# Corleno/Nonstationary_Multivariate_Gaussian_Process

Measured on AMD Instinct MI355X. Metric: log-posterior evals/sec (N=2048, D=3 nonseparable GP), higher is better.
Workload: dtype f64

## Files before the change

nonstationary_multivariate_gaussian_process_amd/csrc/nmgp_chol.hip:

```cpp
#include "nmgp_internal.h"
#include <cstring>

namespace nmgpk {

static inline int cdiv_c(long long a, long long b) { return (int)((a + b - 1) / b); }

typedef double v4d __attribute__((ext_vector_type(4)));

#define SY_BM 128
#define SY_BK 16
#define SY_LD (SY_BM + 16)
#define SY_SB 8

__device__ __forceinline__ int clamp_row_pair(int r, int rows) {
    int rc = r < rows - 1 ? r : rows - 2;
    return rc < 0 ? 0 : rc;
}

__device__ __forceinline__ double fast_recip(double p) {
    double x = __builtin_amdgcn_rcp(p);
    double e = fma(-p, x, 1.0);
    x = fma(x, e, x);
    e = fma(-p, x, 1.0);
    x = fma(x, e, x);
// ... 1445 lines not shown
#pragma unroll
        for (int kk = 0; kk < 4; ++kk) x0 = __builtin_amdgcn_mfma_f64_16x16x4f64(ai[kk], T[pp][kk], x0, 0, 0, 0);
        T[pp] = x0;
#pragma unroll
        for (int kk = 0; kk < 4; ++kk)
#pragma unroll
            for (int q = pp + 1; q < 4; ++q) {
                const double a = reinterpret_cast<const double*>(&ops[(q == 1 ? 0 : (q == 2 ? 1 : 3)) + pp][lane])[kk];
                T[q] = __builtin_amdgcn_mfma_f64_16x16x4f64(a, T[pp][kk], T[q], 0, 0, 0);
            }
    }
    if (v0) {
#pragma unroll
        for (int q = 0; q < 4; ++q)
#pragma unroll
            for (int r = 0; r < 4; ++r) A[(size_t)(16 * q + 4 * r + l4) * lda + row] = T[q][r];
    }
}

static void trsm_64(hipStream_t s, const double* L, int ldl, int nb, double* A, int lda, int rows, int batch,
                    long long bstride, bool precise) {
    if (rows <= 0) return;
    if (precise) {
        NMGP_LAUNCH(k_trsm_64, dim3(cdiv_c(rows, 64), batch), dim3(256), 0, s, L, ldl, nb, A, lda, rows, bstride);
    } else if (nb == 64) {
        NMGP_LAUNCH(k_trsm_64h<5>, dim3(cdiv_c(rows, 64), batch), dim3(256), 0, s, L, ldl, A, lda, rows, bstride);
    } else {
        const long long wgs = (long long)cdiv_c(rows, 128) * batch;
        const int reps = wgs >= 4096 ? 4 : (wgs >= 2048 ? 2 : 1);
        NMGP_LAUNCH(k_trsm_64m, dim3(cdiv_c(rows, 128 * reps), batch), dim3(256), 0, s, L, ldl, nb, A, lda, rows, bstride, reps);
    }
}

#define PS_XLD 66
#define PS_XPS_OFF 6656
#define PS_XS_OFF (PS_XPS_OFF + 64 * PS_XLD)
#define PS_SMEM_DOUBLES (PS_XS_OFF + 64 * PS_XLD)

template <int MODE, int OCC = 2>
__global__ __launch_bounds__(512, OCC) void k_panel_step(double* __restrict__ Ab, int lda, int ck, int has_prev_a,
                                                        int has_next_a,
                                                        int m_act, int pend, long long bstride, int* __restrict__ info,
                                                        int istride, int T, int u_mrows, int u_ncols, int u_kflags,
                                                        int u_tiles, int nbatch, int pre_a, int un_fresh, int u_tri,
                                                        long long* __restrict__ stamps) {
    const int has_prev = MODE == 0 ? has_prev_a : (MODE == 2 ? 1 : 0);
    const int has_next = MODE == 0 ? has_next_a : (MODE == 1 ? 1 : 0);
    const int pre = MODE == 0 ? pre_a : 0;
    constexpr int kOpsT = MODE == 1 ? 0 : 4096;
    constexpr int kXps = PS_XPS_OFF;
    constexpr int kXs = MODE == 1 ? 2560 : PS_XS_OFF;
    constexpr int kSmem = MODE == 1 ? 2560 + 64 * PS_XLD
                                    : (MODE == 2 ? 6656 : (PS_SMEM_DOUBLES > 4 * SY_BK * SY_LD ? PS_SMEM_DOUBLES : 4 * SY_BK * SY_LD));
    static_assert(MODE != 1 || sizeof(Potf2Lds) <= kSmem * sizeof(double), "the factorisation's LDS aliases the step's");
#define PS_STAMP(i)                                                              \
    do {                                                                         \
        if (stamps && blockIdx.x == 0 && threadIdx.x == 0) stamps[i] = (long long)wall_clock64(); \
    } while (0)
    PS_STAMP(0);
    __shared__ __attribute__((aligned(32))) double smem[kSmem];
    const int tid = threadIdx.x, lane = tid & 63, w = tid >> 6;
    const int l15 = lane & 15, l4 = lane >> 4;
    const int bx = (int)blockIdx.x / nbatch, by = (int)blockIdx.x - bx * nbatch;
    if (bx >= T) {
        if constexpr (MODE == 0) {
            const int t = bx - T + by * u_tiles;
            const double* Ap = Ab + (size_t)(ck - 64) * lda + (ck + 128);
            double* Cp = Ab + (size_t)(ck + 128) * lda + (ck + 128);
            syrk_tile_body<4, SY_BK>(Ap, lda, Cp, lda, u_mrows, u_ncols, 64, bstride, bstride, u_kflags, -u_tiles, nbatch, t, 0,
                                     0, smem, smem + 2 * SY_BK * SY_LD, u_tri, 0);
        }
        return;
    }
    double* A = Ab + (size_t)by * bstride;
    v4d* opsC = reinterpret_cast<v4d*>(smem);
    v4d* opsT = reinterpret_cast<v4d*>(smem + kOpsT);
    double* Xps = smem + (MODE == 0 ? kXps : 0);
    double* Xs = smem + (MODE == 2 ? 0 : kXs);
    const bool wg0 = bx == 0;
    const bool isC = wg0 && w < 4;
    const bool wg1 = pre && bx == 1;
    const bool isP = wg1 && w < 4;
    const int row = wg0 ? ck + 64 + 16 * w + l15 : ck + 128 + 128 * (bx - 1) + 16 * w + l15;
    const bool rv = row < m_act && !(wg0 && w >= 4);
    const int rowc = row < m_act ? row : (m_act - 1);
    const bool un_used = has_next && (has_prev || wg0);
    double oc[8], ot[5];
    v4d Xp[4], Tk[4], Un[4];
    const double* Lp = A + (size_t)(ck - 64) * lda;
    if (has_prev) {
#pragma unroll
        for (int j = 0; j < 8; ++j) {
            const int e = tid + 512 * j, q = e >> 10, sx = (e >> 6) & 15, l = e & 63;
            oc[j] = -Lp[(size_t)(4 * sx + (l >> 4)) * lda + ck + 16 * q + (l & 15)];
        }
    }
    {
        const double* L = A + (size_t)ck * lda + ck;
#pragma unroll
        for (int j = 0; j < 5; ++j) {
            const int idx = tid + 512 * j;
            const int blk = idx >> 8, kk = (idx >> 6) & 3, l = idx & 63;
            const int rr = l & 15, kc = 4 * kk + (l >> 4);
            double v;
            if (blk < 6) {
                const int q = blk == 0 ? 1 : (blk < 3 ? 2 : 3);
                const int pp = blk == 0 ? 0 : (blk < 3 ? blk - 1 : blk - 3);
                v = -L[(size_t)(16 * pp + kc) * lda + 16 * q + rr];
            } else {
                const int q = blk - 6;
                if (kc < rr) v = L[(size_t)(16 * q + rr) * lda + 16 * q + kc];
                else if (kc == rr) v = 1.0 / L[(size_t)(16 * q + rr) * lda + 16 * q + rr];
                else v = 0.0;
            }
            ot[j] = v;
        }
    }
    auto load_rows = [&]() {
#pragma unroll
        for (int q = 0; q < 4; ++q)
#pragma unroll
            for (int r = 0; r < 4; ++r) {
                const int c = 16 * q + 4 * r + l4;
                Tk[q][r] = rv ? A[(size_t)(ck + c) * lda + rowc] : 0.0;
                Xp[q][r] = (rv && has_prev) ? Lp[(size_t)c * lda + rowc] : 0.0;
                Un[q][r] = (rv && un_used && row < un_fresh) ? A[(size_t)(ck + 64 + c) * lda + rowc] : 0.0;
            }
    };
    if constexpr (MODE != 2) load_rows();
    if (has_prev) {
#pragma unroll
        for (int j = 0; j < 8; ++j) {
            const int e = tid + 512 * j, q = e >> 10, sx = (e >> 6) & 15, l = e & 63;
            smem[((q * 4 + (sx >> 2)) * 64 + l) * 4 + (sx & 3)] = oc[j];
        }
        if (isP) {
#pragma unroll
            for (int q = 0; q < 4; ++q)
#pragma unroll
                for (int r = 0; r < 4; ++r) Xps[(16 * w + l15) * PS_XLD + 16 * q + 4 * r + l4] = Xp[q][r];
        }
    }
#pragma unroll
    for (int j = 0; j < 5; ++j) {
        const int idx = tid + 512 * j;
        const int blk = idx >> 8, kk = (idx >> 6) & 3, l = idx & 63;
        smem[kOpsT + (blk * 64 + l) * 4 + kk] = ot[j];
    }
    if constexpr (MODE == 2) load_rows();
    __syncthreads();
    PS_STAMP(1);
    if (has_prev && has_next && !wg0) {
#pragma unroll
        for (int j = 0; j < 8; ++j) {
            const int e = tid + 512 * j, q = e >> 10, sx = (e >> 6) & 15, l = e & 63;
            oc[j] = -Lp[(size_t)(4 * sx + (l >> 4)) * lda + ck + 64 + 16 * q + (l & 15)];
        }
    }
    if (has_prev && (!wg0 || isC)) {
#pragma unroll
        for (int sg = 0; sg < 4; ++sg)
#pragma unroll
            for (int kk = 0; kk < 4; ++kk)
#pragma unroll
                for (int q = 0; q < 4; ++q) {
                    const double a = reinterpret_cast<const double*>(&opsC[(q * 4 + sg) * 64 + lane])[kk];
                    Tk[q] = __builtin_amdgcn_mfma_f64_16x16x4f64(a, Xp[sg][kk], Tk[q], 0, 0, 0);
                }
    }
    PS_STAMP(2);
#pragma unroll
    for (int pp = 0; pp < 4; ++pp) {
        const v4d ai = opsT[(6 + pp) * 64 + lane];
        v4d x0 = {0.0, 0.0, 0.0, 0.0};
#pragma unroll
        for (int kk = 0; kk < 4; ++kk) x0 = __builtin_amdgcn_mfma_f64_16x16x4f64(ai[kk], Tk[pp][kk], x0, 0, 0, 0);
        Tk[pp] = x0;
#pragma unroll
        for (int kk = 0; kk < 4; ++kk)
#pragma unroll
            for (int q = pp + 1; q < 4; ++q) {
                const double a = reinterpret_cast<const double*>(&opsT[((q == 1 ? 0 : (q == 2 ? 1 : 3)) + pp) * 64 + lane])[kk];
                Tk[q] = __builtin_amdgcn_mfma_f64_16x16x4f64(a, Tk[pp][kk], Tk[q], 0, 0, 0);
            }
    }
    if (rv) {
#pragma unroll
        for (int q = 0; q < 4; ++q)
#pragma unroll
            for (int r = 0; r < 4; ++r) A[(size_t)(ck + 16 * q + 4 * r + l4) * lda + row] = Tk[q][r];
    }
    PS_STAMP(3);
    if (!has_next) return;
    if (!wg0) {
        if (isP) {
#pragma unroll
            for (int q = 0; q < 4; ++q)
#pragma unroll
                for (int r = 0; r < 4; ++r) Xs[(16 * w + l15) * PS_XLD + 16 * q + 4 * r + l4] = Tk[q][r];
        }
        if (wg1 && !has_prev) __syncthreads();
        if (has_prev) {
            __syncthreads();
#pragma unroll
            for (int j = 0; j < 8; ++j) {
                const int e = tid + 512 * j, q = e >> 10, sx = (e >> 6) & 15, l = e & 63;
                smem[((q * 4 + (sx >> 2)) * 64 + l) * 4 + (sx & 3)] = oc[j];
            }
            __syncthreads();
#pragma unroll
            for (int sg = 0; sg < 4; ++sg)
#pragma unroll
                for (int kk = 0; kk < 4; ++kk)
#pragma unroll
                    for (int q = 0; q < 4; ++q) {
                        const double a = reinterpret_cast<const double*>(&opsC[(q * 4 + sg) * 64 + lane])[kk];
                        Un[q] = __builtin_amdgcn_mfma_f64_16x16x4f64(a, Xp[sg][kk], Un[q], 0, 0, 0);
                    }
        }
        if (rv && (has_prev || row >= un_fresh)) {
#pragma unroll
            for (int q = 0; q < 4; ++q)
#pragma unroll
                for (int r = 0; r < 4; ++r) A[(size_t)(ck + 64 + 16 * q + 4 * r + l4) * lda + row] = Un[q][r];
        }
        if (isP) {
#pragma unroll 1
            for (int q0 = 0; q0 < 4; q0 += 2) {
                v4d Vn[2];
#pragma unroll
                for (int qq = 0; qq < 2; ++qq)
#pragma unroll
                    for (int r = 0; r < 4; ++r) Vn[qq][r] = A[(size_t)(ck + 128 + 16 * (q0 + qq) + 4 * r + l4) * lda + rowc];
                if (has_prev) {
#pragma unroll
                    for (int sg = 0; sg < 4; ++sg)
#pragma unroll
                        for (int kk = 0; kk < 4; ++kk)
#pragma unroll
                            for (int qq = 0; qq < 2; ++qq) {
                                const double a = -Xps[(16 * (q0 + qq) + l15) * PS_XLD + 16 * sg + 4 * kk + l4];
                                const double b = Xps[(16 * w + l15) * PS_XLD + 16 * sg + 4 * kk + l4];
                                Vn[qq] = __builtin_amdgcn_mfma_f64_16x16x4f64(a, b, Vn[qq], 0, 0, 0);
                            }
                }
#pragma unroll
                for (int sg = 0; sg < 4; ++sg)
#pragma unroll
                    for (int kk = 0; kk < 4; ++kk)
#pragma unroll
                        for (int qq = 0; qq < 2; ++qq) {
                            const double a = -Xs[(16 * (q0 + qq) + l15) * PS_XLD + 16 * sg + 4 * kk + l4];
                            const double b = Xs[(16 * w + l15) * PS_XLD + 16 * sg + 4 * kk + l4];
                            Vn[qq] = __builtin_amdgcn_mfma_f64_16x16x4f64(a, b, Vn[qq], 0, 0, 0);
                        }
#pragma unroll
                for (int qq = 0; qq < 2; ++qq)
#pragma unroll
                    for (int r = 0; r < 4; ++r) A[(size_t)(ck + 128 + 16 * (q0 + qq) + 4 * r + l4) * lda + row] = Vn[qq][r];
            }
        }
        return;
    }
    if (isC) {
#pragma unroll
        for (int q = 0; q < 4; ++q)
#pragma unroll
            for (int r = 0; r < 4; ++r) Xs[(16 * w + l15) * PS_XLD + 16 * q + 4 * r + l4] = Tk[q][r];
    }
    PS_STAMP(4);
    __syncthreads();
    PS_STAMP(5);
    if (isC) {
#pragma unroll
        for (int sg = 0; sg < 4; ++sg)
#pragma unroll
            for (int kk = 0; kk < 4; ++kk)
#pragma unroll
                for (int q = 0; q < 4; ++q) {
                    const double a = -Xs[(16 * q + l15) * PS_XLD + 16 * sg + 4 * kk + l4];
                    Un[q] = __builtin_amdgcn_mfma_f64_16x16x4f64(a, Tk[sg][kk], Un[q], 0, 0, 0);
                }
    }
    Potf2Lds& P = *reinterpret_cast<Potf2Lds*>(smem);
    __syncthreads();
    if (isC) {
#pragma unroll
        for (int q = 0; q < 4; ++q)
#pragma unroll
            for (int r = 0; r < 4; ++r) {
                const int rr = 16 * w + l15, cc = 16 * q + 4 * r + l4;
                P.S[cc * PB_LD + rr] = (cc <= rr) ? Un[q][r] : 0.0;
            }
    }
    __syncthreads();
    PS_STAMP(6);
    potf2b_core_mfma(P, info + (size_t)by * istride, ck + 64);
    PS_STAMP(7);
    potf2b_store(A + (size_t)(ck + 64) * lda + (ck + 64), lda, 64, P, tid, 512);
    PS_STAMP(8);
#undef PS_STAMP
}

__global__ void k_set_row(double* __restrict__ A, int lda, int row, const double* __restrict__ v, int n,
                          long long bstride, long long vstride, int cps) {
    int j = blockIdx.x * blockDim.x + threadIdx.x;
    if (j < n) A[(size_t)blockIdx.y * bstride + (size_t)j * lda + row] = v[(size_t)(blockIdx.y / cps) * vstride + j];
}
void set_row(hipStream_t s, double* A, int lda, int row, const double* v, int n, int batch, long long bstride,
             long long vstride, int cps) {
    NMGP_LAUNCH(k_set_row, dim3(cdiv_c(n, 256), batch), dim3(256), 0, s, A, lda, row, v, n, bstride, vstride, cps < 1 ? 1 : cps);
}
__global__ void k_get_row(const double* __restrict__ A, int lda, int row, double* __restrict__ v, int n,
                          long long bstride, long long vstride) {
    int j = blockIdx.x * blockDim.x + threadIdx.x;
    if (j < n) v[(size_t)blockIdx.y * vstride + j] = A[(size_t)blockIdx.y * bstride + (size_t)j * lda + row];
}
void get_row(hipStream_t s, const double* A, int lda, int row, double* v, int n, int batch, long long bstride,
             long long vstride) {
    NMGP_LAUNCH(k_get_row, dim3(cdiv_c(n, 256), batch), dim3(256), 0, s, A, lda, row, v, n, bstride, vstride);
}

struct Factorisation {
    hipStream_t s, s2;
    double* A;
    int lda, n, extra, xtri;
    int* info;
    int batch;
    long long bs;
    int is;
    bool precise;
    const SyrkHook* hook;
    long long* stamps;
    bool block_done = false;

    double* at(int row, int col) const { return A + (size_t)col * lda + row; }
    int active_rows(int cend) const { return n + extra + (cend < xtri ? cend : xtri); }
    bool take_block_done() {
        const bool done = block_done;
        block_done = false;
        return done;
    }

    void update(hipStream_t st, int c0, int k, int c1, int ncols, int fuse_width) {
        const bool fuse = fuse_width >= 64 && !precise;
        const bool done = syrk_lower(st, at(c1, c0), lda, at(c1, c1), lda, active_rows(c0 + k) - c1, ncols, k, batch, bs, -1, 0,
                                     xtri > 0 ? n + extra - c1 : kNoTriRows, c0, fuse ? info : nullptr, is, c1, hook);
        if (fuse) block_done = done;
    }

    void block_solve(int c0, int w) {
        if (!take_block_done()) potf2_64(s, at(c0, c0), lda, w, info, c0, batch, bs, is, precise);
        trsm_64(s, at(c0, c0), lda, w, at(c0 + w, c0), lda, active_rows(c0 + w) - (c0 + w), batch, bs, precise);
    }

    void fused_steps(int c0, int w, bool leaf) {
        if (!take_block_done()) potf2_64(s, at(c0, c0), lda, 64, info, c0, batch, bs, is, precise);
        const int nk = w / 64;
        for (int k = 0; k < nk; ++k) {
            const int ck = c0 + 64 * k;
            const int m_act = active_rows(ck + 64);
            const int rows = m_act - (ck + 64);
            if (rows <= 0) continue;
            const int has_prev = k > 0, has_next = k + 1 < nk;
            const int T = 1 + (rows > 64 ? cdiv_c(rows - 64, 128) : 0);
            SyrkPlan pl;
            const int u_m = m_act - (ck + 128), u_n = c0 + w - (ck + 128);
            if (has_prev && u_m > 0 && u_n > 0) pl = syrk_plan(lda, lda, u_m, u_n, 64, 1, 0, true);
            const int pre = (ck + 192 <= c0 + w) ? 1 : 0;
            if (pre) pl.kflags |= 128;
            long long* st = stamps ? stamps + (size_t)(ck / 64) * 16 : nullptr;
            const int un_fresh = xtri > 0 ? n + extra + (has_prev ? ck - 64 : ck) : kNoTriRows;
            const int u_tri = xtri > 0 ? n + extra - 64 * NMGP_XTRI_SEED_BLOCKS : kNoTriRows;
            if (leaf && pl.tiles == 0 && !pre && nk == 2) {
                if (k == 0)
                    NMGP_LAUNCH((k_panel_step<1, 4>), dim3((unsigned)(T * batch)), dim3(512), 0, s, A, lda, ck, 0, 1, m_act, c0 + w, bs, info,
                                is, T, 0, 0, 0, 0, batch, 0, un_fresh, u_tri, st);
                else
                    NMGP_LAUNCH((k_panel_step<2, 6>), dim3((unsigned)(T * batch)), dim3(512), 0, s, A, lda, ck, 1, 0, m_act, c0 + w, bs, info,
                                is, T, 0, 0, 0, 0, batch, 0, un_fresh, u_tri, st);
            } else {
                NMGP_LAUNCH((k_panel_step<0, 2>), dim3((unsigned)((T + pl.tiles) * batch)), dim3(512), 0, s, A, lda, ck, has_prev, has_next, m_act,
                            c0 + w, bs, info, is, T, pl.mrows, u_n, pl.kflags, pl.tiles, batch, pre, un_fresh, u_tri, st);
            }
        }
    }

    void panel_rl(int c0, int w) {
        for (int j0 = c0; j0 < c0 + w; j0 += 64) {
            const int jb = (c0 + w - j0 < 64) ? (c0 + w - j0) : 64;
            block_solve(j0, jb);
            update(s, j0, jb, j0 + jb, c0 + w - (j0 + jb), c0 + w - (j0 + jb));
        }
    }

    enum Leaf {
        kBlockSolve,
        kFusedSteps,
        kLeaf128
    };
    void panel_halving(int c0, int w, int base, Leaf leaf) {
        if (w <= base) {
            if (leaf == kBlockSolve || (leaf == kLeaf128 && w != 128)) block_solve(c0, w);
            else fused_steps(c0, w, leaf == kLeaf128);
            return;
        }
        int h = ((w / 2 + 63) / 64) * 64;
        if (h >= w) h = ((w - 1) / 64) * 64;
        panel_halving(c0, h, base, leaf);
        update(s, c0, h, c0 + h, w - h, w - h);
        panel_halving(c0 + h, w - h, base, leaf);
    }

    void panel(int c0, int w) {
        const Switches& sw = switches();
        const bool mfma_ok = w > 0 && (w % 64 == 0) && (lda % 2 == 0) && !precise;
        const bool small = sw.fused_max_batch >= 0 ? batch <= sw.fused_max_batch : (long long)batch * n <= 73728;
        const int rec_min_batch = 4;
        if (mfma_ok && (sw.panel == Switches::kFused || (sw.panel == Switches::kAuto && small)))
            panel_halving(c0, w, fused_base(w), kFusedSteps);
        else if (mfma_ok && sw.panel == Switches::kAuto && batch >= rec_min_batch && w >= 128)
            panel_halving(c0, w, 128, kLeaf128);
        else if (sw.panel == Switches::kRl || (sw.panel != Switches::kRec && batch < rec_min_batch))
            panel_rl(c0, w);
        else
            panel_halving(c0, w, 64, kBlockSolve);
    }
    int fused_base(int w) const {
        if (switches().fused_base >= 64) return switches().fused_base;
        if (w > 256 && (batch >= 16 || (xtri > 0 && batch >= 5))) return 256;
        return w;
    }

    void run(int nb1, hipEvent_t* ev) {
        const bool la = (s2 != nullptr && ev != nullptr && n > 2 * nb1 && batch <= switches().la_max_batch && !precise);
        if (!la) {
            for (int c0 = 0; c0 < n; c0 += nb1) {
                const int w1 = (n - c0 < nb1) ? (n - c0) : nb1;
                const int c1 = c0 + w1;
                panel(c0, w1);
                update(s, c0, w1, c1, n - c1, n - c1 < nb1 ? n - c1 : nb1);
            }
            return;
        }
        hipEventRecord(ev[0], s);
        hipStreamWaitEvent(s2, ev[0], 0);
        int k = 0;
        bool prevB = false;
        for (int c0 = 0; c0 < n; c0 += nb1, ++k) {
            const int w1 = (n - c0 < nb1) ? (n - c0) : nb1;
            const int c1 = c0 + w1;
            const int w1n = (c1 < n) ? ((n - c1 < nb1) ? (n - c1) : nb1) : 0;
            const int c2 = c1 + w1n;
            hipEvent_t evPanel = ev[1 + 2 * k], evB = ev[2 + 2 * k];
            panel(c0, w1);
            if (c1 >= n) break;
            if (prevB) hipStreamWaitEvent(s, ev[2 + 2 * (k - 1)], 0);
            update(s, c0, w1, c1, w1n, w1n);
            hipEventRecord(evPanel, s);
            prevB = false;
            if (c2 < n) {
                hipStreamWaitEvent(s2, evPanel, 0);
                update(s2, c0, w1, c2, n - c2, 0);
                hipEventRecord(evB, s2);
                prevB = true;
            }
        }
        if (prevB) hipStreamWaitEvent(s, ev[2 + 2 * (k - 1)], 0);
    }
};

void potrf_lower(hipStream_t s, hipStream_t s2, hipEvent_t* ev, double* A, int lda, int n, int extra, int xtri,
                 int nb1, int* info, int batch, long long bstride, int istride, const SyrkHook* hook, int precise) {
    if (nb1 <= 0)
        nb1 = (batch >= 16 && n >= 4096) ? 2048
              : (((batch >= 4 && n >= 4096) || (batch >= 32 && n >= 2048)) && (long long)batch * n > 73728) ? 1024 : 512;
    const int nsteps = (n + 63) / 64;
    Factorisation f{s, s2, A, lda, n, extra, xtri, info, batch, bstride, istride, precise != 0, hook, g_step_stamps.begin(s, nsteps)};
    f.run(nb1, ev);
    g_step_stamps.dump(s, nsteps);
}

static_assert(SY_BM + 2 * SY_BK - 2 <= 64 * NMGP_XTRI_SEED_BLOCKS, "update tiles of L^-T rows would read left of the seeded band");
static_assert(NMGP_XTRI_SEED_BLOCKS == 3, "k_panel_step (u_tri) and k_xtri_seed's grid (4 column blocks per row block) assume three seeded blocks");
__global__ __launch_bounds__(256) void k_xtri_seed(double* __restrict__ A, int lda, int row0, int n, int pad,
                                                    long long bstride) {
    A += (size_t)blockIdx.z * bstride;
    const int lane = threadIdx.x & 63, w = threadIdx.x >> 6;
    if (blockIdx.x == gridDim.x - 1) {
        for (int c = blockIdx.y * 256 + threadIdx.x; c < n; c += 256 * gridDim.y)
            for (int q = 0; q < pad; ++q) A[(size_t)c * lda + row0 + q] = 0.0;
        return;
    }
    const int b = blockIdx.x;
    const int r = 64 * b + lane;
    const int cb = b - NMGP_XTRI_SEED_BLOCKS + (int)blockIdx.y;
    if (cb < 0 || r >= n) return;
#pragma unroll 4
    for (int k = 0; k < 16; ++k) {
        const int c = 64 * cb + w + 4 * k;
        if (c < n) A[(size_t)c * lda + row0 + pad + r] = (r == c) ? 1.0 : 0.0;
    }
}
void identity_rows(hipStream_t s, double* A, int lda, int row0, int n, int pad, int batch, long long bstride) {
    NMGP_LAUNCH(k_xtri_seed, dim3(cdiv_c(n, 64) + 1, NMGP_XTRI_SEED_BLOCKS + 1, batch), dim3(256), 0, s, A, lda, row0, n, pad, bstride);
}

}
```

Baseline: 1690.

## Add fused 256-column leaf panel using left-looking MFMA step kernels

Adds a k_leaf_step kernel that, for each 64-column block, applies the catch-up update from earlier in-panel blocks, does the triangular solve and optionally factorises the next diagonal block with f64 MFMA, all in one launch. When the recursive kLeaf128 panel reaches width 256, it now runs a sequence of four such launches instead of splitting into two 128 leaves with a separate trailing update. This is meant to cut kernel launches and intermediate global traffic, at the cost of redundant catch-up reads and higher register/LDS pressure, with occupancy hints tuned per step.

```diff
diff --git a/nonstationary_multivariate_gaussian_process_amd/csrc/nmgp_chol.hip b/nonstationary_multivariate_gaussian_process_amd/csrc/nmgp_chol.hip
--- a/nonstationary_multivariate_gaussian_process_amd/csrc/nmgp_chol.hip
+++ b/nonstationary_multivariate_gaussian_process_amd/csrc/nmgp_chol.hip
@@ -1771,6 +1771,209 @@
 #undef PS_STAMP
 }
 
+template <int NP, bool FACT, int OCC>
+__global__ __launch_bounds__(512, OCC) void k_leaf_step(double* __restrict__ Ab, int lda, int ck, int m_act, long long bstride,
+                                                       int* __restrict__ info, int istride, int T, int nbatch, int t_fresh0,
+                                                       int t_fresh1) {
+    constexpr int kOpsC = 2560;
+    constexpr int kSmem = kOpsC + (FACT ? 64 * PS_XLD : 4096);
+    static_assert(64 * PS_XLD >= 4096, "Xs aliases (and covers) the catch-up operands");
+    static_assert(!FACT || sizeof(Potf2Lds) <= kSmem * sizeof(double), "the factorisation's LDS aliases the step's");
+    static_assert(64 * NP <= 64 * NMGP_XTRI_SEED_BLOCKS, "the catch-up of a row of L^-T would read left of the seeded band");
+    __shared__ __attribute__((aligned(32))) double smem[kSmem];
+    const int tid = threadIdx.x, lane = tid & 63, w = tid >> 6;
+    const int l15 = lane & 15, l4 = lane >> 4;
+    const int bx = (int)blockIdx.x / nbatch, by = (int)blockIdx.x - bx * nbatch;
+    double* A = Ab + (size_t)by * bstride;
+    v4d* opsT = reinterpret_cast<v4d*>(smem);
+    v4d* opsC = reinterpret_cast<v4d*>(smem + kOpsC);
+    double* Xs = smem + kOpsC;
+    const bool wg0 = bx == 0;
+    const bool isC = wg0 && w < 4;
+    const int row = wg0 ? ck + 64 + 16 * w + l15 : ck + 128 + 128 * (bx - 1) + 16 * w + l15;
+    const bool rv = row < m_act && !(wg0 && w >= 4);
+    const int rowc = row < m_act ? row : (m_act - 1);
+    const bool tload = rv && !(row >= t_fresh0 && row < t_fresh1);
+    const int wu = __builtin_amdgcn_readfirstlane(w);
+    const unsigned vrow = (unsigned)(l4 * lda + rowc), vops = (unsigned)(l4 * lda + l15);
+    auto colp = [&](int col) { return A + (size_t)col * lda; };
+    double oc[8], ot[5];
+    v4d Xp[4], Tk[4];
+    auto load_ops = [&](int p) {
+        const int cb = ck - 64 * (NP - p);
+#pragma unroll
+        for (int j = 0; j < 8; ++j) oc[j] = -(colp(cb + 4 * (wu + 8 * (j & 1))) + ck + 16 * (j >> 1))[vops];
+    };
+    auto store_ops = [&]() {
+#pragma unroll
+        for (int j = 0; j < 8; ++j) smem[kOpsC + (((j >> 1) * 4 + (j & 1) * 2 + (wu >> 2)) * 64 + lane) * 4 + (wu & 3)] = oc[j];
+    };
+    auto load_x = [&](int p) {
+        const int cb = ck - 64 * (NP - p);
+#pragma unroll
+        for (int q = 0; q < 4; ++q) Xp[q] = v4d{0.0, 0.0, 0.0, 0.0};
+        if (rv) {
+#pragma unroll
+            for (int q = 0; q < 4; ++q)
+#pragma unroll
+                for (int r = 0; r < 4; ++r) Xp[q][r] = colp(cb + 16 * q + 4 * r)[vrow];
+        }
+    };
+    load_ops(0);
+    {
+        const double* L = A + (size_t)ck * lda + ck;
+#pragma unroll
+        for (int j = 0; j < 5; ++j) {
+            const int idx = tid + 512 * j;
+            const int blk = idx >> 8, kk = (idx >> 6) & 3, l = idx & 63;
+            const int rr = l & 15, kc = 4 * kk + (l >> 4);
+            double v;
+            if (blk < 6) {
+                const int q = blk == 0 ? 1 : (blk < 3 ? 2 : 3);
+                const int pp = blk == 0 ? 0 : (blk < 3 ? blk - 1 : blk - 3);
+                v = -L[(size_t)(16 * pp + kc) * lda + 16 * q + rr];
+            } else {
+                const int q = blk - 6;
+                if (kc < rr) v = L[(size_t)(16 * q + rr) * lda + 16 * q + kc];
+                else if (kc == rr) v = 1.0 / L[(size_t)(16 * q + rr) * lda + 16 * q + rr];
+                else v = 0.0;
+            }
+            ot[j] = v;
+        }
+    }
+    store_ops();
+#pragma unroll
+    for (int j = 0; j < 5; ++j) {
+        const int idx = tid + 512 * j;
+        const int blk = idx >> 8, kk = (idx >> 6) & 3, l = idx & 63;
+        smem[(blk * 64 + l) * 4 + kk] = ot[j];
+    }
+#pragma unroll
+    for (int q = 0; q < 4; ++q) Tk[q] = v4d{0.0, 0.0, 0.0, 0.0};
+    if (tload) {
+#pragma unroll
+        for (int q = 0; q < 4; ++q)
+#pragma unroll
+            for (int r = 0; r < 4; ++r) Tk[q][r] = colp(ck + 16 * q + 4 * r)[vrow];
+    }
+    load_x(0);
+    __syncthreads();
+#pragma unroll
+    for (int p = 0; p < NP; ++p) {
+        if (!wg0 || isC) {
+#pragma unroll
+            for (int sg = 0; sg < 4; ++sg)
+#pragma unroll
+                for (int kk = 0; kk < 4; ++kk)
+#pragma unroll
+                    for (int q = 0; q < 4; ++q) {
+                        const double a = reinterpret_cast<const double*>(&opsC[(q * 4 + sg) * 64 + lane])[kk];
+                        Tk[q] = __builtin_amdgcn_mfma_f64_16x16x4f64(a, Xp[sg][kk], Tk[q], 0, 0, 0);
+                    }
+        }
+        if (p + 1 < NP) {
+            __syncthreads();
+            load_ops(p + 1);
+            if constexpr (OCC > 4) {
+                store_ops();
+                __builtin_amdgcn_sched_barrier(0);
+                load_x(p + 1);
+            } else {
+                load_x(p + 1);
+                store_ops();
+            }
+            __syncthreads();
+        }
+    }
+#pragma unroll
+    for (int pp = 0; pp < 4; ++pp) {
+        const v4d ai = opsT[(6 + pp) * 64 + lane];
+        v4d x0 = {0.0, 0.0, 0.0, 0.0};
+#pragma unroll
+        for (int kk = 0; kk < 4; ++kk) x0 = __builtin_amdgcn_mfma_f64_16x16x4f64(ai[kk], Tk[pp][kk], x0, 0, 0, 0);
+        Tk[pp] = x0;
+#pragma unroll
+        for (int kk = 0; kk < 4; ++kk)
+#pragma unroll
+            for (int q = pp + 1; q < 4; ++q) {
+                const double a = reinterpret_cast<const double*>(&opsT[((q == 1 ? 0 : (q == 2 ? 1 : 3)) + pp) * 64 + lane])[kk];
+                Tk[q] = __builtin_amdgcn_mfma_f64_16x16x4f64(a, Tk[pp][kk], Tk[q], 0, 0, 0);
+            }
+    }
+    if (rv) {
+#pragma unroll
+        for (int q = 0; q < 4; ++q)
+#pragma unroll
+            for (int r = 0; r < 4; ++r) colp(ck + 16 * q + 4 * r)[vrow] = Tk[q][r];
+    }
+    if constexpr (FACT) {
+        if (!wg0) return;
+        v4d Un[4];
+        if (isC) {
+#pragma unroll
+            for (int q = 0; q < 4; ++q)
+#pragma unroll
+                for (int r = 0; r < 4; ++r) Un[q][r] = colp(ck + 64 + 16 * q + 4 * r)[vrow];
+        }
+#pragma unroll 1
+        for (int p = 0; p < NP; ++p) {
+            const int cb = ck - 64 * (NP - p);
+#pragma unroll
+            for (int j = 0; j < 8; ++j) oc[j] = colp(cb + wu + 8 * j)[ck + 64 + lane];
+            __syncthreads();
+#pragma unroll
+            for (int j = 0; j < 8; ++j) Xs[lane * PS_XLD + wu + 8 * j] = oc[j];
+            __syncthreads();
+            if (isC) {
+#pragma unroll
+                for (int sg = 0; sg < 4; ++sg)
+#pragma unroll
+                    for (int kk = 0; kk < 4; ++kk) {
+                        const double b = Xs[(16 * w + l15) * PS_XLD + 16 * sg + 4 * kk + l4];
+#pragma unroll
+                        for (int q = 0; q < 4; ++q) {
+                            const double a = -Xs[(16 * q + l15) * PS_XLD + 16 * sg + 4 * kk + l4];
+                            Un[q] = __builtin_amdgcn_mfma_f64_16x16x4f64(a, b, Un[q], 0, 0, 0);
+                        }
+                    }
+            }
+        }
+        __syncthreads();
+        if (isC) {
+#pragma unroll
+            for (int q = 0; q < 4; ++q)
+#pragma unroll
+                for (int r = 0; r < 4; ++r) Xs[(16 * w + l15) * PS_XLD + 16 * q + 4 * r + l4] = Tk[q][r];
+        }
+        __syncthreads();
+        if (isC) {
+#pragma unroll
+            for (int sg = 0; sg < 4; ++sg)
+#pragma unroll
+                for (int kk = 0; kk < 4; ++kk)
+#pragma unroll
+                    for (int q = 0; q < 4; ++q) {
+                        const double a = -Xs[(16 * q + l15) * PS_XLD + 16 * sg + 4 * kk + l4];
+                        Un[q] = __builtin_amdgcn_mfma_f64_16x16x4f64(a, Tk[sg][kk], Un[q], 0, 0, 0);
+                    }
+        }
+        Potf2Lds& P = *reinterpret_cast<Potf2Lds*>(smem);
+        __syncthreads();
+        if (isC) {
+#pragma unroll
+            for (int q = 0; q < 4; ++q)
+#pragma unroll
+                for (int r = 0; r < 4; ++r) {
+                    const int rr = 16 * w + l15, cc = 16 * q + 4 * r + l4;
+                    P.S[cc * PB_LD + rr] = (cc <= rr) ? Un[q][r] : 0.0;
+                }
+        }
+        __syncthreads();
+        potf2b_core_mfma(P, info + (size_t)by * istride, ck + 64);
+        potf2b_store(A + (size_t)(ck + 64) * lda + (ck + 64), lda, 64, P, tid, 512);
+    }
+}
+
 __global__ void k_set_row(double* __restrict__ A, int lda, int row, const double* __restrict__ v, int n,
                           long long bstride, long long vstride, int cps) {
     int j = blockIdx.x * blockDim.x + threadIdx.x;
@@ -1855,6 +2058,32 @@
         }
     }
 
+    void leaf256(int c0) {
+        if (!take_block_done()) potf2_64(s, at(c0, c0), lda, 64, info, c0, batch, bs, is, precise);
+        const int f0 = xtri > 0 ? n + extra + c0 : kNoTriRows;
+        for (int k = 0; k < 4; ++k) {
+            const int ck = c0 + 64 * k;
+            const int m_act = active_rows(ck + 64);
+            const int rows = m_act - (ck + 64);
+            if (rows <= 0) continue;
+            const int T = 1 + (rows > 64 ? cdiv_c(rows - 64, 128) : 0);
+            const dim3 grid((unsigned)(T * batch));
+            if (k == 0)
+                NMGP_LAUNCH((k_panel_step<1, 4>), grid, dim3(512), 0, s, A, lda, ck, 0, 1, m_act, c0 + 128, bs, info, is, T, 0, 0, 0, 0, batch,
+                            0, f0, xtri > 0 ? n + extra - 64 * NMGP_XTRI_SEED_BLOCKS : kNoTriRows,
+                            stamps ? stamps + (size_t)(ck / 64) * 16 : nullptr);
+            else if (k == 1)
+                NMGP_LAUNCH((k_leaf_step<1, true, 4>), grid, dim3(512), 0, s, A, lda, ck, m_act, bs, info, is, T, batch, kNoTriRows,
+                            kNoTriRows);
+            else if (k == 2)
+                NMGP_LAUNCH((k_leaf_step<2, true, 4>), grid, dim3(512), 0, s, A, lda, ck, m_act, bs, info, is, T, batch, f0,
+                            xtri > 0 ? f0 + 128 : kNoTriRows);
+            else
+                NMGP_LAUNCH((k_leaf_step<3, false, 6>), grid, dim3(512), 0, s, A, lda, ck, m_act, bs, info, is, T, batch, f0,
+                            xtri > 0 ? f0 + 192 : kNoTriRows);
+        }
+    }
+
     void panel_rl(int c0, int w) {
         for (int j0 = c0; j0 < c0 + w; j0 += 64) {
             const int jb = (c0 + w - j0 < 64) ? (c0 + w - j0) : 64;
@@ -1872,6 +2101,10 @@
         if (w <= base) {
             if (leaf == kBlockSolve || (leaf == kLeaf128 && w != 128)) block_solve(c0, w);
             else fused_steps(c0, w, leaf == kLeaf128);
+            return;
+        }
+        if (leaf == kLeaf128 && w == 256) {
+            leaf256(c0);
             return;
         }
         int h = ((w / 2 + 63) / 64) * 64;
```

Measured after the change: 1709, median of 6. 1.01x the previous value.
